# ddrakard/tensorflow-distributed-on-gke

Hardware: AMD Instinct MI355X
Metric: tokens/sec (whole node), Transformer-base en-pt at 1/2/4/8 MI355X (higher is better)
Workload: dtype bf16; 1 GPU; model=transformer-base (6L, d_model=512, heads=8, d_ff=2048, vocab 7765/7010), global_batch=64, local_batch=64, seq_len=128, parallelism=dp1, hip_graph=single, grad_comm=fp32, defer_wgrad=True

## Files before the change

### csrc/kernels/attn_bwd.h

```cpp
#pragma once
#include "attn_impl.h"

namespace tdg {

#define TDG_ATTENDS(key, q, klim, Lq, causal) \
  (((key) < (klim)) & ((q) < (Lq)) & (!(causal) | ((key) <= (q))))
#define TDG_PDS_KEY_LANE(U_, full, sv, dpv, lse, del, c, key, q4, klim, Lq, causal, p, ds)   \
  if (full) {                                                                                \
    _Pragma("unroll") for (int r_ = 0; r_ < 4; ++r_)                                         \
    _Pragma("unroll") for (int u_ = 0; u_ < U_; ++u_) {                                      \
      const float pv_ = fast_exp2((sv)[u_][r_] * (c) - (lse)[r_]);                           \
      (p)[u_][r_] = pv_;                                                                     \
      (ds)[u_][r_] = pv_ * ((dpv)[u_][r_] - (del)[r_]);                                      \
    }                                                                                        \
  } else {                                                                                   \
    _Pragma("unroll") for (int r_ = 0; r_ < 4; ++r_) {                                       \
      const int q_ = (q4) + r_;                                                              \
      _Pragma("unroll") for (int u_ = 0; u_ < U_; ++u_) {                                    \
        const bool ok_ = TDG_ATTENDS((key)[u_], q_, klim, Lq, causal);                       \
        const float pv_ = masked_exp2((sv)[u_][r_] * (c) - (lse)[r_], ok_);                  \
        (p)[u_][r_] = pv_;                                                                   \
        (ds)[u_][r_] = pv_ * ((dpv)[u_][r_] - (del)[r_]);                                    \
      }                                                                                      \
    }                                                                                        \
// ... 598 lines not shown
#pragma unroll
      for (int ks = 0; ks < T::KS; ++ks) {
#pragma unroll
        for (int u = 0; u < U; ++u) {
          sv[u] = mfma16(kfr[cb][ks], qf[u][ks], sv[u]);
          dpv[u] = mfma16(vfr[cb][ks], of[u][ks], dpv[u]);
        }
      }
      const int ks0 = k0 + 16 * t;
      const bool full = qminw + 16 * U <= a.Lq && ks0 + 15 < klim && (!causal || ks0 + 15 <= qminw);
      TDG_DS_QUERY_LANE(U, full, sv, dpv, L, D, c, qrow, ks0 + 4 * g, klim, a.Lq, causal, ds[tt])
      if constexpr (tt == 1) {
#pragma unroll
        for (int u = 0; u < U; ++u)
          dsf[u][s2] = pack8(ds[0][u], ds[1][u]);
      }
    });
    uint32_t ktra[T::DT];
#pragma unroll
    for (int dt = 0; dt < T::DT; ++dt) ktra[dt] = slotK + troff[dt];
    short4_t klo[2], khi[2];
    T::template frag_tr_at<0>(ktra[0], klo[0], khi[0]);
    static_for<2 * T::DT>([&](auto ic) {
      constexpr int i = decltype(ic)::value, s2 = i / T::DT, dt = i % T::DT, cb = i & 1, nb = cb ^ 1;
      if constexpr (i + 1 < 2 * T::DT) {
        T::template frag_tr_at<(i + 1) / T::DT>(ktra[(i + 1) % T::DT], klo[nb], khi[nb]);
        lgkm_wait<2>();
      } else {
        lgkm_wait<0>();
      }
      tie(klo[cb]);
      tie(khi[cb]);
      const short8_t kt2 = cat4(klo[cb], khi[cb]);
#pragma unroll
      for (int u = 0; u < U; ++u) dq[u][dt] = mfma16(kt2, dsf[u][s2], dq[u][dt]);
    });
  }
  wait_vmcnt<0>();
  if (!a.skip_bf16) {
#pragma unroll
  for (int u = 0; u < U; ++u) {
    TDG_STORE_GRAD_ROW(T::DT, a.dq, a.dq_sb, a.dq_sl, a.dq_sh, b, h, qrow[u], a.Lq, dq[u], a.scale, g)
  }
  }
  if (a.dq8) {
    float* prow = a.cs_part ? a.cs_part + ((long long)b * a.cs_np + xb) * a.cs_ld + h * 64 + a.cs_q
                            : nullptr;
    attn_emit_g8<U>(dq, a.scale, qrow, a.Lq, a.dq8 + b * a.dq_sb + h * a.dq_sh, a.dq_sl, a.sg8[0],
                    a.amaxg8, prow, reinterpret_cast<float*>(smem), lane, w);
  }
}

struct DsImg {
  static constexpr int RB = 256;
  __device__ static __forceinline__ int off(int row, int byte) {
    const int seg = (byte >> 5) ^ (row & 7);
    return row * RB + (seg << 5) + ((byte & 31) ^ (((row >> 3) & 1) << 4));
  }
  __device__ static __forceinline__ short8_t frag_tr(const char* lds, int s2, int dt, int lane) {
    const int g = lane >> 4, w = lane & 15, q = w >> 2, p = w & 3;
    const int r1 = 32 * s2 + 4 * g + q;
    const int byte = (16 * dt + 4 * p) * 2;
    return cat4(lds_read_tr(lds + off(r1, byte)), lds_read_tr(lds + off(r1 + 16, byte)));
  }
};

constexpr int FDO_STAGES = 3, FDO_SB = (128 + 64) * BK * 2;
__device__ __forceinline__ void fdo_tile(const AttnArgs& a, int b, int h, char* smem, int wid,
                                         int lane, f32x4 (&acc)[2][2]) {
  constexpr int NW = 8, BM = 128, BN = 64, WN = 2, TM = 2, TN = 2, STAGES = FDO_STAGES;
  constexpr int A_BYTES = BM * BK * 2, SB = FDO_SB;
  using GA = Glds<true, BM, NW>;
  using GB = Glds<false, BN, NW>;
  constexpr int PT = GA::P + GB::P;
  const int wm = wid / WN, wn = wid % WN;
  const int K = a.fdo_d;
  const bf16_t* Y = reinterpret_cast<const bf16_t*>(a.fdo_dy) + (size_t)b * a.Lq * a.fdo_ldy;
  const bf16_t* W = reinterpret_cast<const bf16_t*>(a.fdo_w) + 64 * h;
  GA ga;
  GB gb;
  ga.init(wid, lane);
  gb.init(wid, lane);
  const int nk = K / BK;
#pragma unroll
  for (int i = 0; i < TM; ++i)
#pragma unroll
    for (int j = 0; j < TN; ++j) acc[i][j] = f32x4{0.f, 0.f, 0.f, 0.f};
#pragma unroll
  for (int st = 0; st < STAGES; ++st) {
    if (st < nk) {
      ga.issue(Y, a.fdo_ldy, a.Lq, K, 0, st * BK, smem + st * SB, wid);
      gb.issue(W, a.fdo_ldw, BN, K, 0, st * BK, smem + st * SB + A_BYTES, wid);
    }
  }
  const int abase = wm * (BM / 4), bbase = wn * (BN / WN);
  short8_t fa0[TM], fb0[TN], fa1[TM], fb1[TN];
  if (nk >= STAGES)
    wait_vmcnt<(STAGES - 1) * PT>();
  else
    wait_vmcnt<0>();
  lds_barrier();
#pragma unroll
  for (int i = 0; i < TM; ++i) fa0[i] = frag<true, BM>(smem, abase + 16 * i, 0, lane);
#pragma unroll
  for (int j = 0; j < TN; ++j) fb0[j] = frag<false, BN>(smem + A_BYTES, bbase + 16 * j, 0, lane);
  constexpr int STEP_OPS = TM * frag_ops<true>() + TN * frag_ops<false>();
  auto kstep = [&](int kt, auto modec) {
    constexpr int MODE = decltype(modec)::value;
    const char* st = smem + (kt % STAGES) * SB;
#pragma unroll
    for (int i = 0; i < TM; ++i) fa1[i] = frag<true, BM>(st, abase + 16 * i, 1, lane);
#pragma unroll
    for (int j = 0; j < TN; ++j) fb1[j] = frag<false, BN>(st + A_BYTES, bbase + 16 * j, 1, lane);
    lgkm_wait<STEP_OPS>();
    tie_all(fa0);
    tie_all(fb0);
    prio_hi();
#pragma unroll
    for (int i = 0; i < TM; ++i)
#pragma unroll
      for (int j = 0; j < TN; ++j) acc[i][j] = mfma16(fb0[j], fa0[i], acc[i][j]);
    prio_lo();
    if constexpr (MODE >= 1) {
      if constexpr (MODE >= 2) wait_vmcnt<(STAGES - 2) * PT>();
      else wait_vmcnt<0>();
      lds_barrier();
      const char* nx = smem + ((kt + 1) % STAGES) * SB;
      if constexpr (MODE == 3) {
        char* ns = smem + (kt % STAGES) * SB;
        ga.issue(Y, a.fdo_ldy, a.Lq, K, 0, (kt + STAGES) * BK, ns, wid);
        gb.issue(W, a.fdo_ldw, BN, K, 0, (kt + STAGES) * BK, ns + A_BYTES, wid);
      }
#pragma unroll
      for (int i = 0; i < TM; ++i) fa0[i] = frag<true, BM>(nx, abase + 16 * i, 0, lane);
#pragma unroll
      for (int j = 0; j < TN; ++j) fb0[j] = frag<false, BN>(nx + A_BYTES, bbase + 16 * j, 0, lane);
    } else {
      lgkm_wait<0>();
    }
    tie_all(fa1);
    tie_all(fb1);
    prio_hi();
#pragma unroll
    for (int i = 0; i < TM; ++i)
#pragma unroll
      for (int j = 0; j < TN; ++j) acc[i][j] = mfma16(fb1[j], fa1[i], acc[i][j]);
    prio_lo();
  };
  int kt = 0;
  for (; kt + STAGES < nk; ++kt) kstep(kt, std::integral_constant<int, 3>{});
  if (kt + STAGES - 1 < nk && kt + 1 < nk) kstep(kt++, std::integral_constant<int, 2>{});
  for (; kt + 1 < nk; ++kt) kstep(kt, std::integral_constant<int, 1>{});
  if (kt < nk) kstep(kt, std::integral_constant<int, 0>{});
  lds_barrier();
}

template <int HD, int U, bool FDO = false>
__global__ __launch_bounds__(512 / U) __attribute__((amdgpu_waves_per_eu(U == 1 ? (HD <= 64 ? 4 : 2) : 2))) void attn_bwd_fused_kernel(AttnArgs a) {
  static_assert(!FDO || (HD == 64 && U == 1), "in-kernel dO: hd 64, 8 waves");
  using T = ATile<HD>;
  using TS = DsImg;
  constexpr int R = 128;
  constexpr int NT = 512 / U;
  constexpr int TB = R * T::RB;
  constexpr int SB = R * TS::RB;
  constexpr int ALIAS = 2 * TB >= SB;
  extern __shared__ __attribute__((aligned(16))) char smem[];
  char* ldsQ = smem;
  char* ldsO = smem + TB;
  char* ldsK = smem + 2 * TB;
  char* ldsS = ALIAS ? smem : smem + 3 * TB;
  float* ldsL = reinterpret_cast<float*>(smem + (ALIAS ? 3 * TB : 3 * TB + SB));
  float* ldsD = ldsL + R;
  const int tid = threadIdx.x, lane = tid & 63, g = lane >> 4, cl = lane & 15;
  const int w = __builtin_amdgcn_readfirstlane(tid >> 6);
  const int bh = a.xcd ? xcd_remap(blockIdx.x, gridDim.x) : blockIdx.x;
  const int b = bh / a.H, h = bh % a.H;
  int klim;
  float scl;
  bool causal;
  key_window(a, b, klim, scl, causal);
  const float c = scl * LOG2E;

  TDG_STAMP(0);
  const bf16_t* qb = a.q + b * a.q_sb + h * a.q_sh;
  const bf16_t* ob = a.dout + b * a.do_sb + h * a.do_sh;
  const bf16_t* kbp = a.k + b * a.k_sb + h * a.k_sh;
  const bf16_t* obo = a.o + b * a.o_sb + h * a.o_sh;
  int key[U];
#pragma unroll
  for (int u = 0; u < U; ++u) key[u] = 16 * (U * w + u) + cl;
  short8_t kf[U][T::KS], vf[U][T::KS];
#pragma unroll
  for (int u = 0; u < U; ++u) {
    const int krow = min(key[u], a.Lk - 1);
    const bf16_t* kp = kbp + (long long)krow * a.k_sl;
    const bf16_t* vp = a.v + b * a.v_sb + (long long)krow * a.v_sl + h * a.v_sh;
    TDG_LOAD_ROW_FRAGS2(HD, lane, key[u] < a.Lk, kf[u], kp, vf[u], vp)
  }
  {
    constexpr int CPR = HD / 8;
    constexpr int TOTAL = R * CPR;
    constexpr int NI = (TOTAL + NT - 1) / NT;
    short8_t vq[NI], vo[NI], vk[NI], vx[NI];
    const short8_t z = {0, 0, 0, 0, 0, 0, 0, 0};
#pragma unroll
    for (int i = 0; i < NI; ++i) {
      const int id = tid + i * NT;
      const int row = id / CPR, cc = id % CPR;
      vq[i] = vo[i] = vk[i] = vx[i] = z;
      if constexpr (TOTAL % NT == 0) {
        const int rq = min(row, a.Lq - 1), rk = min(row, a.Lk - 1);
        vq[i] = ld8_or0(qb + (long long)rq * a.q_sl + cc * 8, row < a.Lq);
        if constexpr (!FDO) vo[i] = ld8_or0(ob + (long long)rq * a.do_sl + cc * 8, row < a.Lq);
        vx[i] = ld8_or0(obo + (long long)rq * a.o_sl + cc * 8, row < a.Lq);
        vk[i] = ld8_or0(kbp + (long long)rk * a.k_sl + cc * 8, row < a.Lk);
      } else {
        if (id < TOTAL && row < a.Lq) {
          vq[i] = *reinterpret_cast<const short8_t*>(qb + (long long)row * a.q_sl + cc * 8);
          if constexpr (!FDO) vo[i] = *reinterpret_cast<const short8_t*>(ob + (long long)row * a.do_sl + cc * 8);
          vx[i] = *reinterpret_cast<const short8_t*>(obo + (long long)row * a.o_sl + cc * 8);
        }
        if (id < TOTAL && row < a.Lk)
          vk[i] = *reinterpret_cast<const short8_t*>(kbp + (long long)row * a.k_sl + cc * 8);
      }
    }
    const float lse_v = (tid < R && tid < a.Lq) ? a.lse[((long long)b * a.H + h) * a.Lq + tid] : INFINITY;
    if constexpr (FDO) {
      f32x4 acc[2][2];
      fdo_tile(a, b, h, smem, w, lane, acc);
      const int wm = w / 2, wn = w % 2;
#pragma unroll
      for (int i = 0; i < 2; ++i)
#pragma unroll
        for (int j = 0; j < 2; ++j) {
          const int m = 32 * wm + 16 * i + cl, n = 32 * wn + 16 * j + 4 * g;
          short4_t o;
#pragma unroll
          for (int r = 0; r < 4; ++r) o[r] = m < a.Lq ? (short)f2bf(acc[i][j][r]) : (short)0;
          *reinterpret_cast<short4_t*>(ldsO + T::off(m, n * 2)) = o;
        }
      __syncthreads();
#pragma unroll
      for (int i = 0; i < NI; ++i) {
        const int id = tid + i * NT;
        const int row = id / CPR, cc = id % CPR;
        if (id < TOTAL) vo[i] = *reinterpret_cast<const short8_t*>(ldsO + T::off(row, cc * 16));
      }
    }
#pragma unroll
    for (int i = 0; i < NI; ++i) {
      const int id = tid + i * NT;
      const int row = id / CPR, cc = id % CPR;
      if (id < TOTAL) {
        *reinterpret_cast<short8_t*>(ldsQ + T::off(row, cc * 16)) = vq[i];
        if constexpr (!FDO) *reinterpret_cast<short8_t*>(ldsO + T::off(row, cc * 16)) = vo[i];
        *reinterpret_cast<short8_t*>(ldsK + T::off(row, cc * 16)) = vk[i];
      }
      float d = 0.f;
#pragma unroll
      for (int e = 0; e < 8; ++e) d += bf2f((bf16_t)vo[i][e]) * bf2f((bf16_t)vx[i][e]);
#pragma unroll
      for (int o = 1; o < CPR; o <<= 1) d += __shfl_xor(d, o, 64);
      if (id < TOTAL && cc == 0) ldsD[row] = row < a.Lq ? d : 0.f;
    }
    if (tid < R) ldsL[tid] = lse_v;
  }
  __syncthreads();
  TDG_STAMP(1);

  f32x4 dk[U][T::DT], dv[U][T::DT];
  TDG_ZERO2(U, T::DT, dk, dv)
  uint32_t pk[U][8][2], dk2[U][8][2];
  const bool active = 16 * U * w < klim;
  if (active) {
#pragma unroll
    for (int t = 0; t < 8; ++t) {
      const bool live = 16 * t < a.Lq && (!causal || 16 * t + 15 >= 16 * U * w);
      if (!live) {
#pragma unroll
        for (int u = 0; u < U; ++u) pk[u][t][0] = pk[u][t][1] = dk2[u][t][0] = dk2[u][t][1] = 0u;
        continue;
      }
      f32x4 sv[U], dpv[U];
#pragma unroll
      for (int u = 0; u < U; ++u) sv[u] = dpv[u] = f32x4{0.f, 0.f, 0.f, 0.f};
#pragma unroll
      for (int ks = 0; ks < T::KS; ++ks) {
        const short8_t qfr = T::frag_row(ldsQ, 16 * t, ks, lane);
        const short8_t ofr = T::frag_row(ldsO, 16 * t, ks, lane);
#pragma unroll
        for (int u = 0; u < U; ++u) {
          sv[u] = mfma16(qfr, kf[u][ks], sv[u]);
          dpv[u] = mfma16(ofr, vf[u][ks], dpv[u]);
        }
      }
      const f32x4 l4 = *reinterpret_cast<const f32x4*>(ldsL + 16 * t + 4 * g);
      const f32x4 d4 = *reinterpret_cast<const f32x4*>(ldsD + 16 * t + 4 * g);
      const int kmaxw = 16 * U * (w + 1) - 1;
      const bool full = kmaxw < klim && 16 * t + 15 < a.Lq && (!causal || kmaxw <= 16 * t);
#pragma unroll
      for (int u = 0; u < U; ++u) {
        float pv[4], dv4[4];
        if (full) {
#pragma unroll
          for (int r = 0; r < 4; ++r) {
            pv[r] = fast_exp2(sv[u][r] * c - l4[r]);
            dv4[r] = pv[r] * (dpv[u][r] - d4[r]);
          }
        } else {
#pragma unroll
          for (int r = 0; r < 4; ++r) {
            const int q = 16 * t + 4 * g + r;
            const bool ok = TDG_ATTENDS(key[u], q, klim, a.Lq, causal);
            pv[r] = masked_exp2(sv[u][r] * c - l4[r], ok);
            dv4[r] = pv[r] * (dpv[u][r] - d4[r]);
          }
        }
        pk[u][t][0] = pack2bf(pv[0], pv[1]);
        pk[u][t][1] = pack2bf(pv[2], pv[3]);
        dk2[u][t][0] = pack2bf(dv4[0], dv4[1]);
        dk2[u][t][1] = pack2bf(dv4[2], dv4[3]);
      }
    }
#pragma unroll
    for (int s2 = 0; s2 < 4; ++s2) {
      if (32 * s2 >= a.Lq) break;
      short8_t pf[U], dsf[U];
#pragma unroll
      for (int u = 0; u < U; ++u) {
        pf[u] = __builtin_bit_cast(short8_t, make_uint4(pk[u][2 * s2][0], pk[u][2 * s2][1],
                                                        pk[u][2 * s2 + 1][0], pk[u][2 * s2 + 1][1]));
        dsf[u] = __builtin_bit_cast(short8_t, make_uint4(dk2[u][2 * s2][0], dk2[u][2 * s2][1],
                                                         dk2[u][2 * s2 + 1][0], dk2[u][2 * s2 + 1][1]));
      }
#pragma unroll
      for (int dt = 0; dt < T::DT; ++dt) {
        const short8_t otr = T::frag_tr(ldsO, s2, dt, lane);
        const short8_t qtr = T::frag_tr(ldsQ, s2, dt, lane);
#pragma unroll
        for (int u = 0; u < U; ++u) {
          dv[u][dt] = mfma16(otr, pf[u], dv[u][dt]);
          dk[u][dt] = mfma16(qtr, dsf[u], dk[u][dt]);
        }
      }
    }
  } else {
#pragma unroll
    for (int u = 0; u < U; ++u)
#pragma unroll
      for (int t = 0; t < 8; ++t) dk2[u][t][0] = dk2[u][t][1] = 0u;
  }
  TDG_STAMP(2);
  __syncthreads();
#pragma unroll
  for (int u = 0; u < U; ++u)
#pragma unroll
    for (int t = 0; t < 8; ++t)
      *reinterpret_cast<uint2*>(ldsS + TS::off(key[u], (16 * t + 4 * g) * 2)) = make_uint2(dk2[u][t][0], dk2[u][t][1]);
  const float sc = a.scale;
#pragma unroll
  for (int u = 0; u < U; ++u) {
    const bool ok = key[u] < a.Lk;
    bf16_t* dkp = a.dk + b * a.dk_sb + (long long)key[u] * a.dk_sl + h * a.dk_sh;
    bf16_t* dvp = a.dv + b * a.dv_sb + (long long)key[u] * a.dv_sl + h * a.dv_sh;
    uint32_t lo[T::DT], hi[T::DT];
    TDG_PACK_STORE_ROW(T::DT, lo, hi, dkp, dk[u], sc, g, ok)
    TDG_PACK_STORE_ROW(T::DT, lo, hi, dvp, dv[u], 1.f, g, ok)
  }
  __syncthreads();

  if (16 * U * w >= a.Lq) return;
  f32x4 dq[U][T::DT];
  TDG_ZERO(U, T::DT, dq)
#pragma unroll
  for (int s2 = 0; s2 < 4; ++s2) {
    if (32 * s2 >= klim) break;
    short8_t dsf[U];
#pragma unroll
    for (int u = 0; u < U; ++u) dsf[u] = TS::frag_tr(ldsS, s2, U * w + u, lane);
#pragma unroll
    for (int dt = 0; dt < T::DT; ++dt) {
      const short8_t ktr = T::frag_tr(ldsK, s2, dt, lane);
#pragma unroll
      for (int u = 0; u < U; ++u) dq[u][dt] = mfma16(ktr, dsf[u], dq[u][dt]);
    }
  }
#pragma unroll
  for (int u = 0; u < U; ++u) {
    const int qrow = 16 * (U * w + u) + cl;
    TDG_STORE_GRAD_ROW(T::DT, a.dq, a.dq_sb, a.dq_sl, a.dq_sh, b, h, qrow, a.Lq, dq[u], sc, g)
  }
#ifdef TDG_STAMPS
  TDG_STAMP(3);
  asm volatile("s_waitcnt vmcnt(0)" ::: "memory");
  TDG_STAMP(4);
#endif
}

#undef TDG_ATTENDS
#undef TDG_PDS_KEY_LANE
#undef TDG_DS_QUERY_LANE

}

using namespace tdg;

namespace {
template <int HD>
constexpr int fused_bwd_lds() {
  constexpr int TB = 128 * HD * 2, SB = 128 * 256;
  return (2 * TB >= SB ? 3 * TB : 3 * TB + SB) + 2 * 128 * 4;
}
}

extern "C" int tdg_attn_bwd_fdo(const AttnArgs* ap, hipStream_t st) {
  const AttnArgs& a = *ap;
  if (a.Lq > 128 || a.Lk > 128 || a.fdo_d != 64 * a.H || a.fdo_d % BK || a.fdo_ldy % 8 ||
      a.fdo_ldw % 8 || !a.fdo_dy || !a.fdo_w)
    return -1;
  constexpr int lds = fused_bwd_lds<64>() > FDO_STAGES * FDO_SB ? fused_bwd_lds<64>() : FDO_STAGES * FDO_SB;
  big_lds<attn_bwd_fused_kernel<64, 1, true>>();
  hipLaunchKernelGGL((attn_bwd_fused_kernel<64, 1, true>), dim3(a.B * a.H), dim3(512), lds, st, a);
  return 0;
}

namespace {
template <int HD>
int bwd_hd(const AttnArgs& a, hipStream_t st) {
  if (a.Lq <= 128 && a.Lk <= 128) {
    constexpr int lds = fused_bwd_lds<HD>();
    constexpr int U = 1;
    big_lds<attn_bwd_fused_kernel<HD, U>>();
    hipLaunchKernelGGL((attn_bwd_fused_kernel<HD, U>), dim3(a.B * a.H), dim3(512 / U), lds, st, a);
    return 0;
  }
  if constexpr (HD == 64) {
    constexpr int U = 2, NS = 4;
    constexpr int lds_dq = NS * 2 * ATile<64>::BYTES;
    constexpr int lds_kv = NS * (2 * ATile<64>::BYTES + 768);
    big_lds<attn_bwd_dq_pipe_kernel<U, NS>>();
    big_lds<attn_bwd_dkdv_pipe_kernel<U, NS>>();
    hipLaunchKernelGGL((attn_bwd_dq_pipe_kernel<U, NS>), dim3(cdiv(a.Lq, 64 * U), a.H, a.B),
                       dim3(256), lds_dq, st, a);
    hipLaunchKernelGGL((attn_bwd_dkdv_pipe_kernel<U, NS>), dim3(cdiv(a.Lk, 64 * U), a.H, a.B),
                       dim3(256), lds_kv, st, a);
    return 0;
  }
  hipLaunchKernelGGL((attn_bwd_dq_kernel<HD, 1>), dim3(cdiv(a.Lq, QB), a.H, a.B), dim3(256),
                     2 * ATile<HD>::BYTES, st, a);
  hipLaunchKernelGGL((attn_bwd_dkdv_kernel<HD, 1>), dim3(cdiv(a.Lk, KB), a.H, a.B), dim3(256),
                     2 * ATile<HD>::BYTES + 2 * QB * 4, st, a);
  return 0;
}
}

extern "C" int tdg_attn_bwd(const AttnArgs* a, int hd, hipStream_t st) {
  TDG_HD_CASES(bwd_hd, *a, st)
}
```

### csrc/kernels/attn_impl.h

```cpp
#pragma once
#include "tdg_api.h"
#include "tdg_common.h"
#include "tdg_attn.h"

#include <cstdlib>
#include "tdg_gemm.h"

namespace tdg {

constexpr float LOG2E = 1.4426950408889634f;
constexpr float LOG2_448 = 8.807354922057604f;

__device__ __forceinline__ float fast_exp2(float x) { return __builtin_amdgcn_exp2f(x); }
__device__ __forceinline__ float masked_exp2(float x, bool ok) {
  float e = fast_exp2(x);
  asm volatile("" : "+v"(e));
  return ok ? e : 0.f;
}

template <int DT>
__device__ __forceinline__ void store_row16(bf16_t* __restrict__ row, const uint32_t (&lo)[DT],
                                            const uint32_t (&hi)[DT], int g, bool store) {
  if constexpr (DT % 2 == 0) {
#pragma unroll
    for (int d = 0; d < DT; d += 2) {
      const auto r0 = __builtin_amdgcn_permlane16_swap(lo[d], lo[d + 1], false, false);
      const auto r1 = __builtin_amdgcn_permlane16_swap(hi[d], hi[d + 1], false, false);
      if (store)
        *reinterpret_cast<uint4*>(row + 16 * (d + (g & 1)) + 8 * (g >> 1)) =
            make_uint4(r0[0], r1[0], r0[1], r1[1]);
    }
  } else {
#pragma unroll
    for (int d = 0; d < DT; ++d)
      if (store) *reinterpret_cast<uint2*>(row + 16 * d + 4 * g) = make_uint2(lo[d], hi[d]);
  }
}
__device__ __forceinline__ void pack_acc(const f32x4& v, float sc, uint32_t& lo, uint32_t& hi) {
  lo = pack2bf(v[0] * sc, v[1] * sc);
  hi = pack2bf(v[2] * sc, v[3] * sc);
}
__device__ __forceinline__ short8_t pack8(const f32x4& x, const f32x4& y) {
  return pack8(x[0], x[1], x[2], x[3], y[0], y[1], y[2], y[3]);
}
#define TDG_ZERO1(N_, x) _Pragma("unroll") for (int i_ = 0; i_ < N_; ++i_) (x)[i_] = f32x4{0.f, 0.f, 0.f, 0.f};
#define TDG_ZERO(U_, N_, x) \
  _Pragma("unroll") for (int u_ = 0; u_ < U_; ++u_) TDG_ZERO1(N_, (x)[u_])
#define TDG_ZERO2(U_, N_, x, y)                                                                   \
  _Pragma("unroll") for (int u_ = 0; u_ < U_; ++u_) _Pragma("unroll") for (int i_ = 0; i_ < N_; ++i_) \
      (x)[u_][i_] = (y)[u_][i_] = f32x4{0.f, 0.f, 0.f, 0.f};

__device__ __forceinline__ short8_t ld8_or0(const bf16_t* p, bool ok) {
  const short8_t v = *reinterpret_cast<const short8_t*>(p);
  const short8_t z = {0, 0, 0, 0, 0, 0, 0, 0};
  return ok ? v : z;
}

__device__ __forceinline__ void key_window(const AttnArgs& a, int b, int& klim, float& scale,
                                           bool& causal) {
  klim = a.Lk;
  scale = a.scale;
  causal = a.causal != 0;
  if (a.kv_len) {
    const int n = a.kv_len[b];
    if (n > 0) {
      klim = min(klim, n);
    } else {
      scale = 0.f;
      causal = false;
    }
  }
}
__device__ __forceinline__ void attn_coords(const AttnArgs& a, int& xb, int& h, int& b) {
  const int gx = gridDim.x, gy = gridDim.y;
  int t = blockIdx.x + gx * (blockIdx.y + gy * blockIdx.z);
  if (a.xcd) t = xcd_remap(t, gx * gy * gridDim.z);
  xb = t % gx;
  h = (t / gx) % gy;
  b = t / (gx * gy);
}
constexpr int QB = 64;
constexpr int KB = 64;

template <int HD>
struct ATile {
  static constexpr int RB = HD * 2;
  static constexpr int SEGS = HD / 16 > 0 ? HD / 16 : 1;
  static constexpr int RPB = 128 / HD;
  static constexpr int BYTES = 64 * RB;
  static constexpr int KS = HD >= 32 ? HD / 32 : 1;
  static constexpr int DT = HD / 16;
  __device__ static __forceinline__ int off(int row, int byte) {
    const int seg = (byte >> 5) ^ ((row / RPB) & (SEGS - 1));
    return row * RB + (seg << 5) + (byte & 31);
  }
  template <int NT = 256>
  struct Chunks {
    static constexpr int CPR = HD / 8;
    static constexpr int TOTAL = 64 * CPR;
    static constexpr int NI = (TOTAL + NT - 1) / NT;
    short8_t v[NI];
  };
  template <int NT = 256>
  __device__ static __forceinline__ void fetch(Chunks<NT>& c, const bf16_t* __restrict__ base,
                                               long long sl, int row0, int nrows, int tid) {
    using C = Chunks<NT>;
#pragma unroll
    for (int i = 0; i < C::NI; ++i) {
      const int id = tid + i * NT;
      const int row = id / C::CPR, cc = id % C::CPR;
      if constexpr (C::TOTAL % NT == 0) {
        const int r = min(row0 + row, nrows - 1);
        c.v[i] = ld8_or0(base + (long long)r * sl + cc * 8, row0 + row < nrows);
      } else {
        c.v[i] = short8_t{0, 0, 0, 0, 0, 0, 0, 0};
        if (id < C::TOTAL && row0 + row < nrows)
          c.v[i] = *reinterpret_cast<const short8_t*>(base + (long long)(row0 + row) * sl + cc * 8);
      }
    }
  }
  template <int NT = 256>
  __device__ static __forceinline__ void put(char* lds, const Chunks<NT>& c, int tid) {
    using C = Chunks<NT>;
#pragma unroll
    for (int i = 0; i < C::NI; ++i) {
      const int id = tid + i * NT;
      if (C::TOTAL % NT != 0 && id >= C::TOTAL) break;
      const int row = id / C::CPR, cc = id % C::CPR;
      *reinterpret_cast<short8_t*>(lds + off(row, cc * 16)) = c.v[i];
    }
  }
  template <int NT = 256>
  __device__ static __forceinline__ void load(char* lds, const bf16_t* __restrict__ base,
                                              long long sl, int row0, int nrows, int tid) {
    Chunks<NT> c;
    fetch<NT>(c, base, sl, row0, nrows, tid);
    put<NT>(lds, c, tid);
  }
  __device__ static __forceinline__ short8_t frag_row(const char* lds, int rbase, int s, int lane) {
// ... 190 lines not shown
```

### csrc/kernels/attn_qkv.h

```cpp
#pragma once
#include "attn_impl.h"

namespace tdg {

template <int STAGES, bool CROSS, bool SB1 = false>
__global__ __launch_bounds__(512) __attribute__((amdgpu_waves_per_eu(SB1 ? 4 : 2))) void qkv_attn_fwd_kernel(
    const QkvAttnArgs qa) {
  constexpr int NW = 8, WM = CROSS ? 4 : 2, WN = CROSS ? 2 : 4, BM = 128, BN = CROSS ? 64 : 192;
  constexpr int NPART = BN / 64;
  constexpr int TM = BM / WM / 16, TN = BN / WN / 16;
  constexpr int A_BYTES = BM * BK * 2, B_BYTES = BN * BK * 2, SB = A_BYTES + B_BYTES;
  using GA = Glds<true, BM, NW>;
  using GB = Glds<true, BN, NW>;
  constexpr int PT = GA::P + GB::P;
  using T = ATile<64>;
  extern __shared__ __attribute__((aligned(16))) char smem[];
  const AttnArgs& a = qa.a;
  const int tid = threadIdx.x, lane = tid & 63;
  const int wid = __builtin_amdgcn_readfirstlane(tid >> 6);
  const int wm = wid / WN, wn = wid % WN;
  const int t = xcd_remap(blockIdx.x, gridDim.x);
  const int h = t % a.H, b = t / a.H;
  const int L = qa.L, d = qa.d, K = d;
  const bf16_t* X = reinterpret_cast<const bf16_t*>(qa.x) + (size_t)b * L * qa.ldx;
  using Ch = typename ATile<64>::template Chunks<512>;
  Ch ck[2], cv[2];
  if constexpr (CROSS) {
    const bf16_t* kb = a.k + b * a.k_sb + h * a.k_sh;
    const bf16_t* vb = a.v + b * a.v_sb + h * a.v_sh;
#pragma unroll
    for (int h64 = 0; h64 < 2; ++h64) {
      ATile<64>::template fetch<512>(ck[h64], kb, a.k_sl, 64 * h64, a.Lk, tid);
      ATile<64>::template fetch<512>(cv[h64], vb, a.v_sl, 64 * h64, a.Lk, tid);
    }
  }

  GA ga;
  GB gb;
  ga.init(wid, lane);
  gb.init(wid, lane);
  int wrow[GB::P];
#pragma unroll
  for (int i = 0; i < GB::P; ++i) wrow[i] = (gb.row[i] >> 6) * d + 64 * h + (gb.row[i] & 63);
  auto issue_b = [&](int k0, char* lds) {
#pragma unroll
    for (int i = 0; i < GB::P; ++i) {
      const long long off = (long long)wrow[i] * qa.ldw + k0 + gb.col[i];
      __builtin_amdgcn_global_load_lds((const void*)(reinterpret_cast<const bf16_t*>(qa.w) + off),
                                       (__attribute__((address_space(3))) void*)(lds + (wid * GB::P + i) * 1024),
                                       16, 0, 0);
    }
  };
  const int nk = K / BK;
  f32x4 acc[TM][TN];
  TDG_ZERO(TM, TN, acc)
#pragma unroll
  for (int st = 0; st < STAGES; ++st) {
    if (st < nk) {
      ga.issue(X, qa.ldx, L, K, 0, st * BK, smem + st * SB, wid);
      issue_b(st * BK, smem + st * SB + A_BYTES);
    }
  }
  const int abase = wm * (BM / WM), bbase = wn * (BN / WN);
  if constexpr (SB1) {
    short8_t fa[TM], fb[TN];
    for (int kt = 0; kt < nk; ++kt) {
      if (kt + 1 < nk) wait_vmcnt<PT>();
      else wait_vmcnt<0>();
      lds_barrier();
      const char* st = smem + (kt % STAGES) * SB;
#pragma unroll
      for (int s2 = 0; s2 < 2; ++s2) {
#pragma unroll
        for (int i = 0; i < TM; ++i) fa[i] = frag<true, BM>(st, abase + 16 * i, s2, lane);
#pragma unroll
        for (int j = 0; j < TN; ++j) fb[j] = frag<true, BN>(st + A_BYTES, bbase + 16 * j, s2, lane);
        lgkm_wait<0>();
        tie_all(fa);
        tie_all(fb);
        prio_hi();
#pragma unroll
        for (int i = 0; i < TM; ++i)
#pragma unroll
          for (int j = 0; j < TN; ++j) acc[i][j] = mfma16(fb[j], fa[i], acc[i][j]);
        prio_lo();
      }
      lds_barrier();
      if (kt + STAGES < nk) {
        char* ns = smem + (kt % STAGES) * SB;
        ga.issue(X, qa.ldx, L, K, 0, (kt + STAGES) * BK, ns, wid);
        issue_b((kt + STAGES) * BK, ns + A_BYTES);
      }
    }
  } else {
  short8_t fa0[TM], fb0[TN], fa1[TM], fb1[TN];
  if (nk >= STAGES)
    wait_vmcnt<(STAGES - 1) * PT>();
  else
    wait_vmcnt<0>();
  lds_barrier();
#pragma unroll
  for (int i = 0; i < TM; ++i) fa0[i] = frag<true, BM>(smem, abase + 16 * i, 0, lane);
#pragma unroll
  for (int j = 0; j < TN; ++j) fb0[j] = frag<true, BN>(smem + A_BYTES, bbase + 16 * j, 0, lane);
  constexpr int STEP_OPS = TM + TN;
  auto kstep = [&](int kt, auto modec) {
    constexpr int MODE = decltype(modec)::value;
    const char* st = smem + (kt % STAGES) * SB;
#pragma unroll
    for (int i = 0; i < TM; ++i) fa1[i] = frag<true, BM>(st, abase + 16 * i, 1, lane);
#pragma unroll
    for (int j = 0; j < TN; ++j) fb1[j] = frag<true, BN>(st + A_BYTES, bbase + 16 * j, 1, lane);
    lgkm_wait<STEP_OPS>();
    tie_all(fa0);
    tie_all(fb0);
    prio_hi();
#pragma unroll
    for (int i = 0; i < TM; ++i)
#pragma unroll
      for (int j = 0; j < TN; ++j) acc[i][j] = mfma16(fb0[j], fa0[i], acc[i][j]);
    prio_lo();
    if constexpr (MODE >= 1) {
      if constexpr (MODE >= 2) wait_vmcnt<(STAGES - 2) * PT>();
      else wait_vmcnt<0>();
      lds_barrier();
      const char* nx = smem + ((kt + 1) % STAGES) * SB;
      if constexpr (MODE == 3) {
        char* ns = smem + (kt % STAGES) * SB;
        ga.issue(X, qa.ldx, L, K, 0, (kt + STAGES) * BK, ns, wid);
        issue_b((kt + STAGES) * BK, ns + A_BYTES);
      }
#pragma unroll
      for (int i = 0; i < TM; ++i) fa0[i] = frag<true, BM>(nx, abase + 16 * i, 0, lane);
#pragma unroll
      for (int j = 0; j < TN; ++j) fb0[j] = frag<true, BN>(nx + A_BYTES, bbase + 16 * j, 0, lane);
// ... 12 lines not shown
  {
    int kt = 0;
    for (; kt + STAGES < nk; ++kt) kstep(kt, std::integral_constant<int, 3>{});
    if (kt + STAGES - 1 < nk && kt + 1 < nk) kstep(kt++, std::integral_constant<int, 2>{});
    for (; kt + 1 < nk; ++kt) kstep(kt, std::integral_constant<int, 1>{});
    if (kt < nk) kstep(kt, std::integral_constant<int, 0>{});
  }
  }
  lds_barrier();

  char* img = smem;
  constexpr int IMG = 2 * T::BYTES;
  const int g = lane >> 4, cl = lane & 15;
  if constexpr (CROSS) {
#pragma unroll
    for (int h64 = 0; h64 < 2; ++h64) {
      ATile<64>::template put<512>(img + IMG + h64 * T::BYTES, ck[h64], tid);
      ATile<64>::template put<512>(img + 2 * IMG + h64 * T::BYTES, cv[h64], tid);
    }
  }
#pragma unroll
  for (int j = 0; j < TN; ++j) {
    const int n = bbase + 16 * j + 4 * g;
    const int part = n >> 6, hc = n & 63;
    const f32x4 bn = *reinterpret_cast<const f32x4*>(qa.bias + part * d + 64 * h + hc);
#pragma unroll
    for (int i = 0; i < TM; ++i) {
      const int m = abase + 16 * i + cl;
      short4_t o;
#pragma unroll
      for (int r = 0; r < 4; ++r) o[r] = (short)f2bf(acc[i][j][r] + bn[r]);
      *reinterpret_cast<short4_t*>(img + part * IMG + T::off(m, hc * 2)) = o;
    }
  }
  __syncthreads();
  {
    const WtBuf wt(qa.qkv, ((size_t)(b + 1) * L * NPART * d) * sizeof(bf16_t));
#pragma unroll
    for (int pass = 0; pass < NPART * 128 * 8 / 512; ++pass) {
      const int id = tid + 512 * pass;
      const int part = id >> 10, row = (id >> 3) & 127, c = id & 7;
      const short8_t v = *reinterpret_cast<const short8_t*>(img + part * IMG + T::off(row, c * 16));
      if (row < L)
        wt.st16(reinterpret_cast<bf16_t*>(qa.qkv) + ((size_t)b * L + row) * NPART * d + part * d + 64 * h + c * 8,
                v);
    }
  }

  const char* ldsQ = img;
  const char* ldsK = img + IMG;
  const char* ldsV = img + 2 * IMG;
  const int w = wid;
  const int qrow = 16 * w + cl;
  int klim;
  float scl;
  bool causal;
  key_window(a, b, klim, scl, causal);
  if (causal) klim = min(klim, 128);
  const float c = scl * LOG2E;
  const int wq0 = 16 * w;
  short8_t qf[T::KS];
#pragma unroll
  for (int s2 = 0; s2 < T::KS; ++s2) qf[s2] = T::frag_row(ldsQ, 16 * w, s2, lane);
  f32x4 oacc[T::DT];
  TDG_ZERO1(T::DT, oacc)
  float m = -INFINITY, l = 0.f;
  constexpr int NT16 = 8;
  if (klim > 0) {
    f32x4 sc[NT16];
#pragma unroll
    for (int tt = 0; tt < NT16; ++tt) {
      sc[tt] = f32x4{0.f, 0.f, 0.f, 0.f};
#pragma unroll
      for (int ks = 0; ks < T::KS; ++ks) sc[tt] = mfma16(T::frag_row(ldsK, 16 * tt, ks, lane), qf[ks], sc[tt]);
    }
    short8_t pf[NT16 / 2];
    softmax_tile<NT16, T::DT>(sc, m, l, oacc, pf, tile_masked(0, 128, klim, causal, wq0), 0, klim, causal,
                              qrow, g, c);
#pragma unroll
    for (int s2 = 0; s2 < NT16 / 2; ++s2)
#pragma unroll
      for (int dt = 0; dt < T::DT; ++dt) oacc[dt] = mfma16(T::frag_tr(ldsV, s2, dt, lane), pf[s2], oacc[dt]);
  }
  TDG_FWD_FINISH(T::DT, a, b, h, qrow, oacc, m, l, g)
}

}

using namespace tdg;

namespace {
template <int STAGES, bool CROSS, bool SB1>
void qkv_attn_launch(const QkvAttnArgs& qa, hipStream_t st) {
  constexpr int SB = (128 + (CROSS ? 64 : 192)) * BK * 2;
  big_lds<qkv_attn_fwd_kernel<STAGES, CROSS, SB1>>();
  hipLaunchKernelGGL((qkv_attn_fwd_kernel<STAGES, CROSS, SB1>), dim3(qa.a.B * qa.a.H), dim3(512),
                     STAGES * SB, st, qa);
}

}
extern "C" int tdg_qkv_attn_fwd(const QkvAttnArgs* qa, hipStream_t st) {
  const AttnArgs& a = qa->a;
  if (qa->L > 128 || qa->L <= 0 || a.Lq != qa->L || a.Lk > 128 || a.Lk <= 0 || qa->d % 64 ||
      qa->d != 64 * a.H || qa->ldx % 8 || qa->ldw % 8 || (!qa->cross && a.Lk != qa->L))
    return -1;
  if (qa->cross)
    qkv_attn_launch<3, true, false>(*qa, st);
  else
    qkv_attn_launch<2, false, true>(*qa, st);
  return 0;
}
```

Measured before the change: 3.713 million tokens/s.

## Use buffer-resource loads and stores with hardware bounds checks in attention kernels

Replaces pointer-based global loads and stores with masked or clamped rows in the fused attention backward and QKV forward kernels. They now go through AMD buffer resource descriptors, whose num_records bound makes out-of-range rows return zero and drops out-of-range stores. This removes per-row clamping, predication and 64-bit address arithmetic, and moves weight DMA to LDS onto buffer_load_lds with a scalar k-offset. In the FDO path, K fragments are now read from LDS after staging instead of being loaded from global memory. Host-side guards on stride and size are added so the 32-bit offsets stay valid.

```diff
diff --git a/csrc/kernels/attn_bwd.h b/csrc/kernels/attn_bwd.h
--- a/csrc/kernels/attn_bwd.h
+++ b/csrc/kernels/attn_bwd.h
@@ -704,16 +704,27 @@
   ga.init(wid, lane);
   gb.init(wid, lane);
   const int nk = K / BK;
+  uint32_t wb[GB::P];
+#pragma unroll
+  for (int i = 0; i < GB::P; ++i) wb[i] = 2u * (uint32_t)(gb.row[i] * a.fdo_ldw + gb.col[i]);
+  const int nrec_w = 2 * ((K - 1) * a.fdo_ldw + BN);
+  const uint32_t kstep_w = 2u * (uint32_t)BK * (uint32_t)a.fdo_ldw;
+  auto issue = [&](int kt, char* lds) {
+    ga.issue(Y, a.fdo_ldy, a.Lq, K, 0, kt * BK, lds, wid);
+#pragma unroll
+    for (int i = 0; i < GB::P; ++i)
+      __builtin_amdgcn_raw_ptr_buffer_load_lds(
+          __builtin_amdgcn_make_buffer_rsrc(const_cast<bf16_t*>(W), (short)0, nrec_w, 0x00020000),
+          (__attribute__((address_space(3))) void*)(lds + A_BYTES + (wid * GB::P + i) * 1024), 16, wb[i],
+          (int)(kstep_w * (uint32_t)kt), 0, 0);
+  };
 #pragma unroll
   for (int i = 0; i < TM; ++i)
 #pragma unroll
     for (int j = 0; j < TN; ++j) acc[i][j] = f32x4{0.f, 0.f, 0.f, 0.f};
 #pragma unroll
   for (int st = 0; st < STAGES; ++st) {
-    if (st < nk) {
-      ga.issue(Y, a.fdo_ldy, a.Lq, K, 0, st * BK, smem + st * SB, wid);
-      gb.issue(W, a.fdo_ldw, BN, K, 0, st * BK, smem + st * SB + A_BYTES, wid);
-    }
+    if (st < nk) issue(st, smem + st * SB);
   }
   const int abase = wm * (BM / 4), bbase = wn * (BN / WN);
   short8_t fa0[TM], fb0[TN], fa1[TM], fb1[TN];
@@ -749,9 +760,7 @@
       lds_barrier();
       const char* nx = smem + ((kt + 1) % STAGES) * SB;
       if constexpr (MODE == 3) {
-        char* ns = smem + (kt % STAGES) * SB;
-        ga.issue(Y, a.fdo_ldy, a.Lq, K, 0, (kt + STAGES) * BK, ns, wid);
-        gb.issue(W, a.fdo_ldw, BN, K, 0, (kt + STAGES) * BK, ns + A_BYTES, wid);
+        issue(kt + STAGES, smem + (kt % STAGES) * SB);
       }
 #pragma unroll
       for (int i = 0; i < TM; ++i) fa0[i] = frag<true, BM>(nx, abase + 16 * i, 0, lane);
@@ -805,20 +814,30 @@
   const float c = scl * LOG2E;
 
   TDG_STAMP(0);
-  const bf16_t* qb = a.q + b * a.q_sb + h * a.q_sh;
-  const bf16_t* ob = a.dout + b * a.do_sb + h * a.do_sh;
-  const bf16_t* kbp = a.k + b * a.k_sb + h * a.k_sh;
-  const bf16_t* obo = a.o + b * a.o_sb + h * a.o_sh;
+  const uint32_t q_slb = 2u * (uint32_t)a.q_sl, k_slb = 2u * (uint32_t)a.k_sl, v_slb = 2u * (uint32_t)a.v_sl;
+  const uint32_t o_slb = 2u * (uint32_t)a.o_sl;
+  const HeadBuf bq(a.q + b * a.q_sb + h * a.q_sh, a.Lq, q_slb, T::RB);
+  const HeadBuf bk(a.k + b * a.k_sb + h * a.k_sh, a.Lk, k_slb, T::RB);
+  const HeadBuf bv(a.v + b * a.v_sb + h * a.v_sh, a.Lk, v_slb, T::RB);
+  const HeadBuf bx(a.o + b * a.o_sb + h * a.o_sh, a.Lq, o_slb, T::RB);
+  const HeadBuf bl(a.lse + ((long long)b * a.H + h) * a.Lq, a.Lq, 4u, 4);
   int key[U];
 #pragma unroll
   for (int u = 0; u < U; ++u) key[u] = 16 * (U * w + u) + cl;
   short8_t kf[U][T::KS], vf[U][T::KS];
 #pragma unroll
   for (int u = 0; u < U; ++u) {
-    const int krow = min(key[u], a.Lk - 1);
-    const bf16_t* kp = kbp + (long long)krow * a.k_sl;
-    const bf16_t* vp = a.v + b * a.v_sb + (long long)krow * a.v_sl + h * a.v_sh;
-    TDG_LOAD_ROW_FRAGS2(HD, lane, key[u] < a.Lk, kf[u], kp, vf[u], vp)
+    const uint32_t ko = (uint32_t)key[u] * k_slb + 16 * g, vo_ = (uint32_t)key[u] * v_slb + 16 * g;
+#pragma unroll
+    for (int s = 0; s < T::KS; ++s) {
+      if constexpr (!FDO) kf[u][s] = bk.ld16(ko + 64 * s);
+      vf[u][s] = bv.ld16(vo_ + 64 * s);
+      if constexpr (HD < 32) {
+        const short8_t z8 = {0, 0, 0, 0, 0, 0, 0, 0};
+        kf[u][s] = g < HD / 8 ? kf[u][s] : z8;
+        vf[u][s] = g < HD / 8 ? vf[u][s] : z8;
+      }
+    }
   }
   {
     constexpr int CPR = HD / 8;
@@ -826,28 +845,21 @@
     constexpr int NI = (TOTAL + NT - 1) / NT;
     short8_t vq[NI], vo[NI], vk[NI], vx[NI];
     const short8_t z = {0, 0, 0, 0, 0, 0, 0, 0};
+    const uint32_t crow = (uint32_t)(tid / CPR), cby = 16u * (uint32_t)(tid % CPR);
 #pragma unroll
     for (int i = 0; i < NI; ++i) {
-      const int id = tid + i * NT;
-      const int row = id / CPR, cc = id % CPR;
-      vq[i] = vo[i] = vk[i] = vx[i] = z;
-      if constexpr (TOTAL % NT == 0) {
-        const int rq = min(row, a.Lq - 1), rk = min(row, a.Lk - 1);
-        vq[i] = ld8_or0(qb + (long long)rq * a.q_sl + cc * 8, row < a.Lq);
-        if constexpr (!FDO) vo[i] = ld8_or0(ob + (long long)rq * a.do_sl + cc * 8, row < a.Lq);
-        vx[i] = ld8_or0(obo + (long long)rq * a.o_sl + cc * 8, row < a.Lq);
-        vk[i] = ld8_or0(kbp + (long long)rk * a.k_sl + cc * 8, row < a.Lk);
-      } else {
-        if (id < TOTAL && row < a.Lq) {
-          vq[i] = *reinterpret_cast<const short8_t*>(qb + (long long)row * a.q_sl + cc * 8);
-          if constexpr (!FDO) vo[i] = *reinterpret_cast<const short8_t*>(ob + (long long)row * a.do_sl + cc * 8);
-          vx[i] = *reinterpret_cast<const short8_t*>(obo + (long long)row * a.o_sl + cc * 8);
-        }
-        if (id < TOTAL && row < a.Lk)
-          vk[i] = *reinterpret_cast<const short8_t*>(kbp + (long long)row * a.k_sl + cc * 8);
-      }
-    }
-    const float lse_v = (tid < R && tid < a.Lq) ? a.lse[((long long)b * a.H + h) * a.Lq + tid] : INFINITY;
+      const uint32_t row = crow + (uint32_t)(i * (NT / CPR));
+      vo[i] = z;
+      vq[i] = bq.ld16(row * q_slb + cby);
+      if constexpr (!FDO) {
+        const HeadBuf bdo(a.dout + b * a.do_sb + h * a.do_sh, a.Lq, 2u * (uint32_t)a.do_sl, T::RB);
+        vo[i] = bdo.ld16(row * (2u * (uint32_t)a.do_sl) + cby);
+      }
+      vx[i] = bx.ld16(row * o_slb + cby);
+      vk[i] = bk.ld16(row * k_slb + cby);
+    }
+    const float lse_l = bl.ld4f(4u * (uint32_t)tid);
+    const float lse_v = tid < a.Lq ? lse_l : INFINITY;
     if constexpr (FDO) {
       f32x4 acc[2][2];
       fdo_tile(a, b, h, smem, w, lane, acc);
@@ -889,12 +901,19 @@
     if (tid < R) ldsL[tid] = lse_v;
   }
   __syncthreads();
+  if constexpr (FDO) {
+#pragma unroll
+    for (int u = 0; u < U; ++u)
+#pragma unroll
+      for (int s = 0; s < T::KS; ++s) kf[u][s] = T::frag_row(ldsK, 16 * (U * w + u), s, lane);
+  }
   TDG_STAMP(1);
 
   f32x4 dk[U][T::DT], dv[U][T::DT];
   TDG_ZERO2(U, T::DT, dk, dv)
   uint32_t pk[U][8][2], dk2[U][8][2];
   const bool active = 16 * U * w < klim;
+  const int kmaxw = 16 * U * (w + 1) - 1;
   if (active) {
 #pragma unroll
     for (int t = 0; t < 8; ++t) {
@@ -919,7 +938,6 @@
       }
       const f32x4 l4 = *reinterpret_cast<const f32x4*>(ldsL + 16 * t + 4 * g);
       const f32x4 d4 = *reinterpret_cast<const f32x4*>(ldsD + 16 * t + 4 * g);
-      const int kmaxw = 16 * U * (w + 1) - 1;
       const bool full = kmaxw < klim && 16 * t + 15 < a.Lq && (!causal || kmaxw <= 16 * t);
 #pragma unroll
       for (int u = 0; u < U; ++u) {
@@ -968,6 +986,7 @@
       }
     }
   } else {
+    TDG_ZERO2(U, T::DT, dk, dv)
 #pragma unroll
     for (int u = 0; u < U; ++u)
 #pragma unroll
@@ -981,23 +1000,26 @@
     for (int t = 0; t < 8; ++t)
       *reinterpret_cast<uint2*>(ldsS + TS::off(key[u], (16 * t + 4 * g) * 2)) = make_uint2(dk2[u][t][0], dk2[u][t][1]);
   const float sc = a.scale;
-#pragma unroll
-  for (int u = 0; u < U; ++u) {
-    const bool ok = key[u] < a.Lk;
-    bf16_t* dkp = a.dk + b * a.dk_sb + (long long)key[u] * a.dk_sl + h * a.dk_sh;
-    bf16_t* dvp = a.dv + b * a.dv_sb + (long long)key[u] * a.dv_sl + h * a.dv_sh;
-    uint32_t lo[T::DT], hi[T::DT];
-    TDG_PACK_STORE_ROW(T::DT, lo, hi, dkp, dk[u], sc, g, ok)
-    TDG_PACK_STORE_ROW(T::DT, lo, hi, dvp, dv[u], 1.f, g, ok)
+  {
+    const uint32_t dk_slb = 2u * (uint32_t)a.dk_sl, dv_slb = 2u * (uint32_t)a.dv_sl;
+    const HeadBuf bdk(a.dk + b * a.dk_sb + h * a.dk_sh, a.Lk, dk_slb, T::RB);
+    const HeadBuf bdv(a.dv + b * a.dv_sb + h * a.dv_sh, a.Lk, dv_slb, T::RB);
+#pragma unroll
+    for (int u = 0; u < U; ++u) {
+      uint32_t lo[T::DT], hi[T::DT];
+      TDG_PACK_STORE_ROW_BUF(T::DT, lo, hi, bdk, (uint32_t)key[u] * dk_slb, dk[u], sc, g)
+      TDG_PACK_STORE_ROW_BUF(T::DT, lo, hi, bdv, (uint32_t)key[u] * dv_slb, dv[u], 1.f, g)
+    }
   }
   __syncthreads();
 
   if (16 * U * w >= a.Lq) return;
   f32x4 dq[U][T::DT];
-  TDG_ZERO(U, T::DT, dq)
+  const int nk2 = (klim + 31) >> 5;
+  const f32x4 zero4 = {0.f, 0.f, 0.f, 0.f};
 #pragma unroll
   for (int s2 = 0; s2 < 4; ++s2) {
-    if (32 * s2 >= klim) break;
+    if (s2 > 0 && s2 >= nk2) break;
     short8_t dsf[U];
 #pragma unroll
     for (int u = 0; u < U; ++u) dsf[u] = TS::frag_tr(ldsS, s2, U * w + u, lane);
@@ -1005,13 +1027,18 @@
     for (int dt = 0; dt < T::DT; ++dt) {
       const short8_t ktr = T::frag_tr(ldsK, s2, dt, lane);
 #pragma unroll
-      for (int u = 0; u < U; ++u) dq[u][dt] = mfma16(ktr, dsf[u], dq[u][dt]);
-    }
-  }
-#pragma unroll
-  for (int u = 0; u < U; ++u) {
-    const int qrow = 16 * (U * w + u) + cl;
-    TDG_STORE_GRAD_ROW(T::DT, a.dq, a.dq_sb, a.dq_sl, a.dq_sh, b, h, qrow, a.Lq, dq[u], sc, g)
+      for (int u = 0; u < U; ++u) dq[u][dt] = mfma16(ktr, dsf[u], s2 == 0 ? zero4 : dq[u][dt]);
+    }
+  }
+  {
+    const uint32_t dq_slb = 2u * (uint32_t)a.dq_sl;
+    const HeadBuf bdq(a.dq + b * a.dq_sb + h * a.dq_sh, a.Lq, dq_slb, T::RB);
+#pragma unroll
+    for (int u = 0; u < U; ++u) {
+      const int qrow = 16 * (U * w + u) + cl;
+      uint32_t lo[T::DT], hi[T::DT];
+      TDG_PACK_STORE_ROW_BUF(T::DT, lo, hi, bdq, (uint32_t)qrow * dq_slb, dq[u], sc, g)
+    }
   }
 #ifdef TDG_STAMPS
   TDG_STAMP(3);
@@ -1034,12 +1061,19 @@
   constexpr int TB = 128 * HD * 2, SB = 128 * 256;
   return (2 * TB >= SB ? 3 * TB : 3 * TB + SB) + 2 * 128 * 4;
 }
+bool fused_bwd_views_ok(const AttnArgs& a, int hd, bool with_dout) {
+  return a.Lq > 0 && a.Lk > 0 && head_stride_ok(a.q_sl, hd) && head_stride_ok(a.k_sl, hd) &&
+         head_stride_ok(a.v_sl, hd) && head_stride_ok(a.o_sl, hd) && head_stride_ok(a.dq_sl, hd) &&
+         head_stride_ok(a.dk_sl, hd) && head_stride_ok(a.dv_sl, hd) &&
+         (!with_dout || head_stride_ok(a.do_sl, hd));
+}
 }
 
 extern "C" int tdg_attn_bwd_fdo(const AttnArgs* ap, hipStream_t st) {
   const AttnArgs& a = *ap;
   if (a.Lq > 128 || a.Lk > 128 || a.fdo_d != 64 * a.H || a.fdo_d % BK || a.fdo_ldy % 8 ||
-      a.fdo_ldw % 8 || !a.fdo_dy || !a.fdo_w)
+      a.fdo_ldw % 8 || !a.fdo_dy || !a.fdo_w || !fused_bwd_views_ok(a, 64, false) ||
+      (long long)a.Lq * a.fdo_ldy >= (1ll << 30) || (long long)a.fdo_d * a.fdo_ldw >= (1ll << 30))
     return -1;
   constexpr int lds = fused_bwd_lds<64>() > FDO_STAGES * FDO_SB ? fused_bwd_lds<64>() : FDO_STAGES * FDO_SB;
   big_lds<attn_bwd_fused_kernel<64, 1, true>>();
@@ -1050,7 +1084,7 @@
 namespace {
 template <int HD>
 int bwd_hd(const AttnArgs& a, hipStream_t st) {
-  if (a.Lq <= 128 && a.Lk <= 128) {
+  if (a.Lq <= 128 && a.Lk <= 128 && fused_bwd_views_ok(a, HD, true)) {
     constexpr int lds = fused_bwd_lds<HD>();
     constexpr int U = 1;
     big_lds<attn_bwd_fused_kernel<HD, U>>();
diff --git a/csrc/kernels/attn_impl.h b/csrc/kernels/attn_impl.h
--- a/csrc/kernels/attn_impl.h
+++ b/csrc/kernels/attn_impl.h
@@ -55,6 +55,53 @@
   const short8_t z = {0, 0, 0, 0, 0, 0, 0, 0};
   return ok ? v : z;
 }
+
+struct HeadBuf {
+  __amdgpu_buffer_rsrc_t r;
+  __device__ __forceinline__ HeadBuf(const void* base, int rows, uint32_t slb, int row_bytes)
+      : r(__builtin_amdgcn_make_buffer_rsrc(const_cast<void*>(base), 0,
+                                             rows > 0 ? (int)((uint32_t)(rows - 1) * slb + (uint32_t)row_bytes) : 0,
+                                             0x00020000)) {}
+  __device__ __forceinline__ short8_t ld16(uint32_t off) const {
+    return __builtin_bit_cast(short8_t, __builtin_amdgcn_raw_buffer_load_b128(r, (int)off, 0, 0));
+  }
+  __device__ __forceinline__ float ld4f(uint32_t off) const {
+    return __builtin_bit_cast(float, __builtin_amdgcn_raw_buffer_load_b32(r, (int)off, 0, 0));
+  }
+  __device__ __forceinline__ void st16(uint32_t off, const uint4& v) const {
+    __builtin_amdgcn_raw_buffer_store_b128(__builtin_bit_cast(u32x4_t, v), r, (int)off, 0, 0);
+  }
+  __device__ __forceinline__ void st8(uint32_t off, const uint2& v) const {
+    __builtin_amdgcn_raw_buffer_store_b64(__builtin_bit_cast(u32x2_t, v), r, (int)off, 0, 0);
+  }
+  __device__ __forceinline__ void st4f(uint32_t off, float v) const {
+    __builtin_amdgcn_raw_buffer_store_b32(__builtin_bit_cast(uint32_t, v), r, (int)off, 0, 0);
+  }
+};
+__host__ __device__ inline bool head_stride_ok(long long sl, int hd) { return sl >= hd && sl < (1ll << 22); }
+
+template <int DT>
+__device__ __forceinline__ void store_row16(const HeadBuf& hb, uint32_t rowoff, const uint32_t (&lo)[DT],
+                                            const uint32_t (&hi)[DT], int g) {
+  if constexpr (DT % 2 == 0) {
+    const uint32_t o = rowoff + 32 * (g & 1) + 16 * (g >> 1);
+#pragma unroll
+    for (int d = 0; d < DT; d += 2) {
+      const auto r0 = __builtin_amdgcn_permlane16_swap(lo[d], lo[d + 1], false, false);
+      const auto r1 = __builtin_amdgcn_permlane16_swap(hi[d], hi[d + 1], false, false);
+      hb.st16(o + 32 * d, make_uint4(r0[0], r1[0], r0[1], r1[1]));
+    }
+  } else {
+#pragma unroll
+    for (int d = 0; d < DT; ++d) hb.st8(rowoff + 32 * d + 8 * g, make_uint2(lo[d], hi[d]));
+  }
+}
+#define TDG_PACK_STORE_ROW_BUF(DT_, lo, hi, hb, rowoff, acc, scale, g)                         \
+  {                                                                                            \
+    _Pragma("unroll") for (int dt_ = 0; dt_ < DT_; ++dt_)                                      \
+        pack_acc((acc)[dt_], scale, lo[dt_], hi[dt_]);              \
+    store_row16<DT_>(hb, rowoff, lo, hi, g);                                                   \
+  }
 
 __device__ __forceinline__ void key_window(const AttnArgs& a, int b, int& klim, float& scale,
                                            bool& causal) {
diff --git a/csrc/kernels/attn_qkv.h b/csrc/kernels/attn_qkv.h
--- a/csrc/kernels/attn_qkv.h
+++ b/csrc/kernels/attn_qkv.h
@@ -2,6 +2,16 @@
 #include "attn_impl.h"
 
 namespace tdg {
+
+template <int P>
+__device__ __forceinline__ void dma_pieces(const uint16_t* base, int nrec, const uint32_t (&off)[P], int soff,
+                                           char* lds, int wid) {
+#pragma unroll
+  for (int i = 0; i < P; ++i)
+    __builtin_amdgcn_raw_ptr_buffer_load_lds(
+        __builtin_amdgcn_make_buffer_rsrc(const_cast<uint16_t*>(base), (short)0, nrec, 0x00020000),
+        (__attribute__((address_space(3))) void*)(lds + (wid * P + i) * 1024), 16, off[i], soff, 0, 0);
+}
 
 template <int STAGES, bool CROSS, bool SB1 = false>
 __global__ __launch_bounds__(512) __attribute__((amdgpu_waves_per_eu(SB1 ? 4 : 2))) void qkv_attn_fwd_kernel(
@@ -42,15 +52,11 @@
   int wrow[GB::P];
 #pragma unroll
   for (int i = 0; i < GB::P; ++i) wrow[i] = (gb.row[i] >> 6) * d + 64 * h + (gb.row[i] & 63);
-  auto issue_b = [&](int k0, char* lds) {
-#pragma unroll
-    for (int i = 0; i < GB::P; ++i) {
-      const long long off = (long long)wrow[i] * qa.ldw + k0 + gb.col[i];
-      __builtin_amdgcn_global_load_lds((const void*)(reinterpret_cast<const bf16_t*>(qa.w) + off),
-                                       (__attribute__((address_space(3))) void*)(lds + (wid * GB::P + i) * 1024),
-                                       16, 0, 0);
-    }
-  };
+  uint32_t wb[GB::P];
+#pragma unroll
+  for (int i = 0; i < GB::P; ++i) wb[i] = 2u * (uint32_t)(wrow[i] * qa.ldw + gb.col[i]);
+  const int nrec_w = 2 * ((NPART * d - 1) * qa.ldw + K);
+  auto issue_b = [&](int k0, char* lds) { dma_pieces<GB::P>(qa.w, nrec_w, wb, 2 * k0, lds, wid); };
   const int nk = K / BK;
   f32x4 acc[TM][TN];
   TDG_ZERO(TM, TN, acc)
@@ -229,7 +235,17 @@
 #pragma unroll
       for (int dt = 0; dt < T::DT; ++dt) oacc[dt] = mfma16(T::frag_tr(ldsV, s2, dt, lane), pf[s2], oacc[dt]);
   }
-  TDG_FWD_FINISH(T::DT, a, b, h, qrow, oacc, m, l, g)
+  {
+    float lu = l;
+    lu = rows_sum(lu);
+    const float inv = softmax_inv(lu);
+    const uint32_t o_slb = 2u * (uint32_t)a.o_sl;
+    const HeadBuf bo(a.out + b * a.o_sb + h * a.o_sh, a.Lq, o_slb, 128);
+    const HeadBuf bl(a.lse + ((long long)b * a.H + h) * a.Lq, a.Lq, 4u, 4);
+    uint32_t lo[T::DT], hi[T::DT];
+    TDG_PACK_STORE_ROW_BUF(T::DT, lo, hi, bo, (uint32_t)qrow * o_slb, oacc, inv, g)
+    if (g == 0) bl.st4f(4u * (uint32_t)qrow, softmax_lse(m, lu));
+  }
 }
 
 }
@@ -249,7 +265,9 @@
 extern "C" int tdg_qkv_attn_fwd(const QkvAttnArgs* qa, hipStream_t st) {
   const AttnArgs& a = qa->a;
   if (qa->L > 128 || qa->L <= 0 || a.Lq != qa->L || a.Lk > 128 || a.Lk <= 0 || qa->d % 64 ||
-      qa->d != 64 * a.H || qa->ldx % 8 || qa->ldw % 8 || (!qa->cross && a.Lk != qa->L))
+      qa->d != 64 * a.H || qa->ldx % 8 || qa->ldw % 8 || (!qa->cross && a.Lk != qa->L) ||
+      !head_stride_ok(a.o_sl, 64) ||
+      (long long)(qa->cross ? 1 : 3) * qa->d * qa->ldw >= (1ll << 30))
     return -1;
   if (qa->cross)
     qkv_attn_launch<3, true, false>(*qa, st);
```

New measurement: 3.725 million tokens/s, median of 6. No clear change (+0.3%).
